# pscoro/JPEG-XL-Lossy-Image-Compression-Thesis

Measured on AMD Instinct MI355X. Metric: MPix/s VarDCT encode @ d1.0, 8K RGB, higher is better.
Workload: dtype f32; 1 GPU; 8k 7680x4320 RGB8 (synth_rgb8), VarDCT d1 e7, cjxl defaults (JXG_FLAGS_CJXL_DEFAULTS: Gaborish + EPF + masking AQ), proposals=0, ans-coded, 1 frame(s) per step, 2 distinct frames cycled, streaming entry points (jxg_submit_rgb8_device / jxg_receive, one host thread); global_batch=1, parallelism=frame-dp1

## Files before the change

jpeg-xl-lossy-image-compression-thesis_amd/csrc/jxg_ac.hip:

```cpp
#include "jxg_device.h"
#include "jxg_kernels.h"

namespace jxg {

constexpr int kAcCtxPad = (kAcCtx + 15) & ~15;
__constant__ __attribute__((aligned(16))) uint8_t c_cluster[kAcCtxPad];

constexpr int kAcThreads = 1024;

struct GroupGeom {
  int bx0, by0, gw, gh;
};
__device__ __forceinline__ uint32_t slot_group(const uint32_t* glist, uint32_t g0, uint32_t i) {
  return glist ? glist[i] : g0 + i;
}
__device__ __forceinline__ GroupGeom group_geom(const AcArgs& a, int g) {
  GroupGeom r;
  const int gx = g % (int)a.gxs, gy = g / (int)a.gxs;
  r.bx0 = gx * 32;
  r.by0 = gy * 32;
  r.gw = min(32, (int)a.bxs - r.bx0);
  r.gh = min(32, (int)a.bys - r.by0);
  return r;
}
// ... 429 lines not shown
}

__device__ __forceinline__ uint32_t wave_incl_scan(uint32_t v) {
  const int lane = threadIdx.x & 63;
#pragma unroll
  for (int d = 1; d < 64; d <<= 1) {
    const uint32_t t = __shfl_up(v, d);
    if (lane >= d) v += t;
  }
  return v;
}
__global__ __launch_bounds__(kAcThreads) void ac_emit_kernel(AcArgs a) {
  __shared__ uint32_t sCode[kMaxClusters * kAcTok];
  __shared__ __attribute__((aligned(16))) uint32_t sBits[kEmitLdsWords];
  __shared__ uint32_t sWave[kAcThreads / 64];
  const int g = (int)slot_group(a.glist, a.g0, blockIdx.x);
  for (int i = threadIdx.x; i < kMaxClusters * kAcTok; i += blockDim.x)
    sCode[i] = a.codes[(i / kAcTok) * kAlpha + (i % kAcTok)];
  for (int i = threadIdx.x; i < kEmitLdsWords / 4; i += blockDim.x)
    reinterpret_cast<uint4*>(sBits)[i] = make_uint4(0, 0, 0, 0);
  const uint32_t n = a.ntok[g * 3] + a.ntok[g * 3 + 1] + a.ntok[g * 3 + 2];
  const uint32_t* rec = a.tokens + (uint64_t)blockIdx.x * kGroupTokStride;
  uint32_t bt[kBands];
#pragma unroll
  for (int i = 0; i < kBands; i++) bt[i] = a.bandtok[g * kBands + i];
  constexpr int kWaves = kAcThreads / 64;
  const int lane = threadIdx.x & 63, wv = threadIdx.x >> 6;
  const uint32_t chunk = ((n + kWaves * 64 - 1) / (kWaves * 64)) * 64;
  const uint32_t lo = min(n, wv * chunk), hi = min(n, lo + chunk);
  __syncthreads();
  auto code_of = [&](uint32_t r) { return sCode[(r & 0xFF) * kAcTok + ((r >> 8) & 63)]; };
  uint32_t tot = 0;
  for (uint32_t k = lo + lane; k < hi; k += 64) {
    const uint32_t r = rec[rec_index(bt, k)];
    tot += (code_of(r) >> 16) + ((r >> 14) & 15);
  }
#pragma unroll
  for (int d = 32; d > 0; d >>= 1) tot += __shfl_xor(tot, d, 64);
  if (lane == 0) sWave[wv] = tot;
  __syncthreads();
  uint32_t run = 0, total = 0;
#pragma unroll
  for (int i = 0; i < kWaves; i++) {
    const uint32_t x = sWave[i];
    run += i < wv ? x : 0u;
    total += x;
  }
  const uint64_t base = a.base[g];
  const bool lds = total <= (uint32_t)kEmitLdsWords * 32u;
  if (!lds) {
    for (uint32_t i = threadIdx.x; i < (total + 31) / 32; i += blockDim.x) a.scratch[(base >> 5) + i] = 0;
    __threadfence();
    __syncthreads();
  }
  uint32_t* buf = lds ? sBits : a.scratch;
  const uint64_t bias = lds ? 0 : base;
  for (uint32_t k0 = lo; k0 < hi; k0 += 64) {
    const uint32_t k = k0 + lane;
    uint32_t len = 0, val = 0;
    if (k < hi) {
      const uint32_t r = rec[rec_index(bt, k)], cl = code_of(r);
      len = (cl >> 16) + ((r >> 14) & 15);
      val = (cl & 0xFFFFu) | ((r >> 18) << (cl >> 16));
    }
    const uint32_t incl = wave_incl_scan(len);
    if (len) {
      const uint64_t pos = bias + run + incl - len;
      const uint64_t w = pos >> 5;
      const uint32_t sh = (uint32_t)(pos & 31);
      atomicOr(&buf[w], val << sh);
      if (sh + len > 32) atomicOr(&buf[w + 1], val >> (32 - sh));
    }
    run += __shfl(incl, 63, 64);
  }
  if (lds) {
    __syncthreads();
    const uint32_t nw = (total + 31) / 32;
    uint32_t* dst = a.scratch + (base >> 5);
    for (uint32_t i = threadIdx.x; i < nw; i += blockDim.x) dst[i] = sBits[i];
  }
  if (threadIdx.x == 0) a.bits[g] = total;
}

#ifndef JXG_ANS_WAVES
#define JXG_ANS_WAVES 8
#endif
constexpr int kAnsWaves = JXG_ANS_WAVES;
__device__ __forceinline__ uint32_t wave_ror1(uint32_t x) {
  return (uint32_t)__builtin_amdgcn_mov_dpp((int)x, 0x13C, 0xF, 0xF, false);
}
__device__ __forceinline__ void ans_chain(const AnsArgs& a, uint32_t blk) {
  __shared__ uint32_t sSym[kAnsHists * 128];
  __shared__ uint32_t sInv[kAnsHists * 4096 / 2];
  __shared__ uint8_t sMap[136];
  const uint32_t* src = reinterpret_cast<const uint32_t*>(a.tab);
  for (uint32_t i = threadIdx.x; i < a.nhist * 128; i += blockDim.x) sSym[i] = src[i];
  for (uint32_t i = threadIdx.x; i < a.nhist * 2048; i += blockDim.x)
    sInv[i] = src[kAnsInvOff / 4 + i];
  for (uint32_t i = threadIdx.x; i < 136; i += blockDim.x) sMap[i] = a.tab[kAnsMapOff + i];
  __syncthreads();
  const uint8_t* inv = reinterpret_cast<const uint8_t*>(sInv);
  const uint32_t lane = threadIdx.x & 63;
  const uint32_t gi = __builtin_amdgcn_readfirstlane(blk * kAnsWaves + (threadIdx.x >> 6));
  if (gi >= a.n) return;
  const uint32_t slot = __builtin_amdgcn_readfirstlane(a.order[gi]);
  const uint32_t g = __builtin_amdgcn_readfirstlane(slot_group(a.glist, a.g0, slot));
  __builtin_amdgcn_s_setprio(3);
  const int n = (int)(a.ntok[g * 3] + a.ntok[g * 3 + 1] + a.ntok[g * 3 + 2]);
  const uint64_t b = (uint64_t)slot * kGroupTokStride;
  uint32_t bt[kBands];
#pragma unroll
  for (int i = 0; i < kBands; i++) bt[i] = a.bandtok[g * kBands + i];
  uint32_t k = 0x130u, v = 0;
  uint32_t rec = (int)lane < min(64, n) ? a.tokens[b + rec_index(bt, n - 1 - lane)] : 0u;
  for (int hi = n; hi > 0; hi -= 64) {
    const int cnt = min(64, hi);
    uint32_t f = 4096, base2 = 0;
    if ((int)lane < cnt) {
      const uint32_t h = sMap[rec & 0xFF], e = sSym[h * 128 + ((rec >> 8) & 63)];
      f = (e & 0xFFF) + 1;
      base2 = 2 * (h * 4096 + (e >> 12));
    }
    const uint32_t Fq = f << 8;
    const uint32_t nf2 = (uint32_t)(-(int)(2 * f));
    const double rcp = 1.0 / (double)f, hr = 0.5 * rcp;
    const int hn = hi - 64;
    const uint32_t nrec = (int)lane < min(64, hn) ? a.tokens[b + rec_index(bt, hn - 1 - lane)] : 0u;
    uint32_t X = 0;
    uint32_t xin = 0;
    auto step = [&](int s) {
      const uint32_t kin = wave_ror1(k);
      const uint32_t sh = kin >= Fq ? 16u : 0u;
      if (s > 0)
        asm("v_cndmask_b32_e64 %0, %1, %2, %3" : "=v"(X) : "v"(X), "v"(xin), "s"(1ull << (s - 1)));
      __builtin_amdgcn_sched_barrier(0);
      const uint32_t vin = wave_ror1(v);
      const uint32_t x = (kin << 12) + vin;
      const uint32_t xs = x >> sh;
      const uint32_t kk = (uint32_t)__builtin_fma((double)xs, rcp, hr);
      const uint32_t x2 = (xs << 1) + base2;
      uint32_t addr;
      asm("v_mad_i32_i24 %0, %1, %2, %3" : "=v"(addr) : "v"(kk), "v"(nf2), "v"(x2));
      v = *reinterpret_cast<const uint16_t*>(inv + addr);
      k = kk;
      xin = x;
      __builtin_amdgcn_sched_barrier(0);
    };
    if (cnt == 64) {
#pragma unroll
      for (int s = 0; s < 64; s++) step(s);
      asm("v_cndmask_b32_e64 %0, %1, %2, %3" : "=v"(X) : "v"(X), "v"(xin), "s"(1ull << 63));
    } else {
      for (int s = 0; s < cnt; s++) {
        const uint32_t kin = wave_ror1(k);
        const bool emit = kin >= Fq;
        const uint32_t t = (kin << 12) >> (emit ? 16 : 0);
        const double P = __builtin_fma((double)t, rcp, hr);
        const uint32_t C = 2 * t + base2;
        const uint32_t vin = wave_ror1(v);
        X = (int)lane == s ? (kin << 12) + vin : X;
        const uint32_t vv = emit ? 0u : vin;
        const uint32_t kk = (uint32_t)__builtin_fma((double)vv, rcp, P);
        const uint32_t addr = (uint32_t)((int)(2 * vv + C) - (int)(2 * f) * (int)kk);
        v = *reinterpret_cast<const uint16_t*>(inv + addr);
        k = kk;
      }
    }
    if ((int)lane < cnt) {
      const bool em = (X >> 20) >= f;
      const uint32_t raw = rec >> 18, nb = (rec >> 14) & 15;
      a.val[b + hi - 1 - lane] = em ? (X & 0xFFFFu) | raw << 16 : raw;
      a.len[b + hi - 1 - lane] = (uint8_t)(em ? nb + 16 : nb);
    }
    rec = nrec;
    if (hi <= 64) {
      const uint32_t kf = __builtin_amdgcn_readlane(k, cnt - 1);
      const uint32_t vf = __builtin_amdgcn_readlane(v, cnt - 1);
      if (lane == 0) a.state[g] = (kf << 12) + vf;
    }
  }
  if (n == 0 && lane == 0) a.state[g] = 0x130000u;
}
__global__ __launch_bounds__(kAnsWaves * 64) void ans_encode_kernel(Batch<AnsArgs> bt_) {
  ans_chain(bt_.a[blockIdx.z], blockIdx.x);
}
constexpr int kSumThreads = 1024;
__global__ __launch_bounds__(kSumThreads) void ans_sums_kernel(Batch<AnsArgs> bt_) {
  __shared__ uint32_t sC[kAnsMaxChunks];
  __shared__ uint32_t sTot[kSumThreads / 64];
  const AnsArgs& a = bt_.a[blockIdx.z];
  const uint32_t slot = blockIdx.x;
  if (slot >= a.n) return;
  const uint32_t g = slot_group(a.glist, a.g0, slot);
  const uint32_t n = a.ntok[g * 3] + a.ntok[g * 3 + 1] + a.ntok[g * 3 + 2];
  const uint32_t K = (n + 63) / 64;
  const uint64_t b = (uint64_t)slot * kGroupTokStride;
  const int lane = threadIdx.x & 63, wv = threadIdx.x >> 6;
  for (uint32_t q = threadIdx.x; q < K; q += kSumThreads) sC[q] = 0;
  __syncthreads();
  const uint32_t off = (64u - (n & 63u)) & 63u, r = n & 15u;
  const uint4* L = reinterpret_cast<const uint4*>(a.len + b);
  for (uint32_t w = threadIdx.x; w < (n + 15) / 16; w += kSumThreads) {
    const uint4 v = L[w];
    const uint32_t d[4] = {v.x, v.y, v.z, v.w};
    const uint32_t valid = min(16u, n - 16u * w);
    uint32_t lo = 0, hi = 0;
#pragma unroll
    for (uint32_t j = 0; j < 16; j++) {
      const uint32_t x = j < valid ? (d[j >> 2] >> (8 * (j & 3))) & 0xFFu : 0u;
      if (j < r) lo += x;
      else hi += x;
    }
    if (lo) atomicAdd(&sC[(16u * w + off) >> 6], lo);
    if (hi) atomicAdd(&sC[(16u * w + r + off) >> 6], hi);
  }
  __syncthreads();
  uint32_t* csum = a.csum + (uint64_t)slot * kAnsMaxChunks;
  uint32_t tot = 0;
  for (uint32_t q = threadIdx.x; q < K; q += kSumThreads) {
    const uint32_t c = sC[q];
    csum[q] = c;
    tot += c;
  }
#pragma unroll
  for (int m = 32; m > 0; m >>= 1) tot += __shfl_xor(tot, m, 64);
  if (lane == 0) sTot[wv] = tot;
  __syncthreads();
  uint32_t total = 32;
#pragma unroll
  for (int i = 0; i < kSumThreads / 64; i++) total += sTot[i];
  if (threadIdx.x == 0) a.bits[g] = total;
  uint32_t* dst = a.scratch + (a.base[g] >> 5);
  for (uint32_t i = threadIdx.x; i < (total + 31) / 32; i += kSumThreads) dst[i] = 0;
}
constexpr int kSegChunks = 64, kEmitThreads = 256;
constexpr int kSegWords = (kSegChunks * 64 * 29 + 31) / 32 + 2;
__global__ __launch_bounds__(kEmitThreads) void ans_emit_kernel(Batch<AnsArgs> bt_) {
  __shared__ __attribute__((aligned(16))) uint32_t sBits[kSegWords];
  __shared__ uint32_t sCs[kSegChunks + 1];
  __shared__ uint32_t sPre[kEmitThreads / 64];
  const AnsArgs& a = bt_.a[blockIdx.z];
  const uint32_t slot = blockIdx.x, seg = blockIdx.y;
  if (slot >= a.n) return;
  const uint32_t g = slot_group(a.glist, a.g0, slot);
  const uint32_t n = a.ntok[g * 3] + a.ntok[g * 3 + 1] + a.ntok[g * 3 + 2];
  const uint32_t K = (n + 63) / 64, q0 = seg * kSegChunks;
  const uint64_t base = a.base[g];
  if (seg == 0 && threadIdx.x == 0) a.scratch[base >> 5] = a.state[g];
  if (q0 >= K) return;
  const uint32_t q1 = min(K, q0 + kSegChunks);
  const uint32_t* csum = a.csum + (uint64_t)slot * kAnsMaxChunks;
  const int lane = threadIdx.x & 63, wv = threadIdx.x >> 6;
  uint32_t pre = 0;
  for (uint32_t q = threadIdx.x; q < q0; q += kEmitThreads) pre += csum[q];
#pragma unroll
  for (int d = 32; d > 0; d >>= 1) pre += __shfl_xor(pre, d, 64);
  if (lane == 0) sPre[wv] = pre;
  if (threadIdx.x <= kSegChunks) sCs[threadIdx.x] = q0 + threadIdx.x < q1 ? csum[q0 + threadIdx.x] : 0u;
  for (int i = threadIdx.x; i < kSegWords; i += kEmitThreads) sBits[i] = 0;
  __syncthreads();
  const uint64_t start = base + 32 + sPre[0] + sPre[1] + sPre[2] + sPre[3];
  const uint32_t sh0 = (uint32_t)(start & 31);
  uint32_t segbits = 0;
  for (uint32_t q = 0; q < q1 - q0; q++) segbits += sCs[q];
  auto chunk_lo = [&](uint32_t q) { return q == 0 ? 0u : n - 64u * (K - q); };
  const uint64_t b = (uint64_t)slot * kGroupTokStride;
  constexpr int kPerWave = kSegChunks / (kEmitThreads / 64);
  uint32_t run = sh0;
  for (int i = 0; i < wv * kPerWave; i++) run += sCs[i];
  for (int i = 0; i < kPerWave; i++) {
    const uint32_t q = q0 + (uint32_t)(wv * kPerWave + i);
    if (q >= q1) break;
    const uint32_t lo = chunk_lo(q), hi = chunk_lo(q + 1);
    const uint32_t k = lo + (uint32_t)lane;
    const uint32_t len = k < hi ? a.len[b + k] : 0u;
    const uint32_t val = k < hi ? a.val[b + k] : 0u;
    const uint32_t incl = wave_incl_scan(len);
    if (len) {
      const uint32_t pos = run + incl - len;
      const uint32_t w = pos >> 5, sh = pos & 31;
      atomicOr(&sBits[w], val << sh);
      if (sh + len > 32) atomicOr(&sBits[w + 1], val >> (32 - sh));
    }
    run += sCs[wv * kPerWave + i];
  }
  __syncthreads();
  const uint32_t nw = (sh0 + segbits + 31) / 32;
  uint32_t* dst = a.scratch + (start >> 5);
  for (uint32_t i = threadIdx.x; i < nw; i += kEmitThreads) {
    const uint32_t v = sBits[i];
    if (i == 0 || i == nw - 1) {
      if (v) atomicOr(&dst[i], v);
    } else {
      dst[i] = v;
    }
  }
}

void launch_ans(const AnsArgs* a, uint32_t k, hipStream_t s) {
  if (!k || !a[0].n) return;
  const Batch<AnsArgs> b = make_batch(a, k);
  uint32_t n = 0, maxtok = 0;
  for (uint32_t i = 0; i < k; i++) {
    n = max(n, a[i].n);
    maxtok = max(maxtok, a[i].max_tokens);
  }
  hipLaunchKernelGGL(ans_encode_kernel, dim3((n + kAnsWaves - 1) / kAnsWaves, 1, k),
                     dim3(kAnsWaves * 64), 0, s, b);
  hipLaunchKernelGGL(ans_sums_kernel, dim3(n, 1, k), dim3(kSumThreads), 0, s, b);
  const uint32_t nseg = (maxtok + kSegChunks * 64 - 1) / (kSegChunks * 64);
  if (nseg) hipLaunchKernelGGL(ans_emit_kernel, dim3(n, nseg, k), dim3(kEmitThreads), 0, s, b);
}

void launch_ac_hist(const AcArgs* a, uint32_t k, uint32_t ngroups, hipStream_t s, bool whole_group) {
  if (!ngroups || !k) return;
  if (whole_group)
    hipLaunchKernelGGL(ac_hist_kernel<32>, dim3(ngroups, 1, k), dim3(1024), 0, s, make_batch(a, k));
  else
    hipLaunchKernelGGL(ac_hist_kernel<8>, dim3(ngroups * kBands, 1, k), dim3(256), 0, s, make_batch(a, k));
}
void launch_ac_emit(const AcArgs& a, uint32_t ngroups, hipStream_t s) {
  if (ngroups) hipLaunchKernelGGL(ac_emit_kernel, dim3(ngroups), dim3(kAcThreads), 0, s, a);
}
hipError_t set_cluster_table(const uint8_t* tab, hipStream_t s) {
  return hipMemcpyToSymbolAsync(HIP_SYMBOL(c_cluster), tab, kAcCtx, 0, hipMemcpyHostToDevice, s);
}

}
```

jpeg-xl-lossy-image-compression-thesis_amd/csrc/jxg_host.cpp:

```cpp
#include <hip/hip_runtime.h>

#include <algorithm>
#include <atomic>
#include <chrono>
#include <cmath>
#include <condition_variable>
#include <cstdio>
#include <cstdlib>
#include <cstring>
#include <deque>
#include <functional>
#include <future>
#include <memory>
#include <mutex>
#include <new>
#include <thread>
#include <vector>

#include "../../include/jxg.h"
#include "jxg_bitstream.h"
#include "jxg_device.h"
#include "jxg_kernels.h"
#include "jxg_helpers.h"
#include "jxg_payload.h"
// ... 1153 lines not shown
    launch_ac_emit(J.aa, J.plan.ng(), s);
    JXG_HIP(hipGetLastError());
    JXG_HIP(hipMemcpyAsync(c->h_gbits.p, c->gbits.p, f.ngroups * 4, hipMemcpyDeviceToHost, s));
    JXG_HIP(hipEventRecord(c->ev[7], s));
  }

  JXG_HIP(hipEventSynchronize(c->ev[2]));
  const Clock::time_point t_lf = Clock::now();
  const size_t nlfcodes = (size_t)nstreams * 4 * kAlpha;
  JXG_HIP(c->h_lfcodes.ensure(nlfcodes));
  uint32_t* lfpacked = c->h_lfcodes.p;
  std::fill(lfpacked, lfpacked + nlfcodes, 0u);
  J.preA.assign(f.nlf, BitWriter());
  J.preB.assign(f.nlf, BitWriter());
  for (uint32_t lg = 0; lg < f.nlf; lg++) {
    if (!J.plan.owns_lf(lg)) continue;
    const uint32_t bx0 = (lg % f.lfxs) * 256, by0 = (lg / f.lfxs) * 256;
    const uint32_t bw = std::min(256u, f.bxs - bx0), bh = std::min(256u, f.bys - by0);
    for (int sidx = 0; sidx < 2; sidx++) {
      const uint32_t sid = lg * 2 + sidx;
      const int nleaves = sidx == 0 ? 3 : 4;
      std::vector<PrefixCode> lc(nleaves);
      for (int l = 0; l < nleaves; l++) {
        lc[l] = build_prefix_code(c->h_lfhist.p + ((size_t)sid * 4 + l) * kAlpha, kAlpha);
        for (int k = 0; k < kAlpha; k++) lfpacked[((size_t)sid * 4 + l) * kAlpha + k] = lc[l].packed(k);
      }
      if (sidx == 0) {
        J.preA[lg].put(2, 0);
        write_modular_prelude(J.preA[lg], kDcTree, 5, 3, lc);
      } else {
        J.preB[lg].put(ceil_log2(bw * bh), c->h_vcount.p[lg] - 1);
        write_modular_prelude(J.preB[lg], (J.lf >> 1) ? kMetaTreeEpf : kMetaTree, 7, 4, lc);
      }
    }
  }
  J.sbase.assign(nstreams, 0);
  cursor = 0;
  for (uint32_t i = 0; i < nstreams; i++) {
    J.sbase[i] = cursor;
    if (J.plan.owns_lf(i / 2)) cursor += ((uint64_t)c->h_sbound.p[i] + 63) & ~31ull;
  }
  const uint64_t lf_words = cursor / 32 + 2;
  JXG_HIP(c->h_sbase.ensure(J.sbase.size()));
  std::copy(J.sbase.begin(), J.sbase.end(), c->h_sbase.p);
  if (J.ans) {
    JXG_HIP(c->scratch.ensure(ac_words + lf_words));
    c->lf_scratch = c->scratch.p + ac_words;
    J.aa.scratch = c->scratch.p;
    JXG_HIP(hipMemcpyAsync(c->up.p + c->up_gbase, c->h_up.p + c->up_gbase,
                           c->up_bytes - c->up_gbase, hipMemcpyHostToDevice, s));
  } else {
    JXG_HIP(c->scratch_lf.ensure(lf_words));
    c->lf_scratch = c->scratch_lf.p;
    JXG_HIP(hipMemcpyAsync(c->up.p + c->up_lf, c->h_up.p + c->up_lf, c->up_bytes - c->up_lf,
                           hipMemcpyHostToDevice, s));
  }
  J.ms_codes = ms_ac_codes + ms_since(t_lf);
  return JXG_OK;
}

static void build_emit(Ctx* c, Job& J) {
  J.la.scratch = c->lf_scratch;
  if (!J.ans) return;
  AnsArgs& na = J.na;
  na = AnsArgs{};
  na.tokens = c->tokens.p;
  na.val = c->tval.p;
  na.len = c->tlen.p;
  na.ntok = c->ntok.p;
  na.bandtok = c->bandtok.p;
  na.tab = c->ans_tab.p;
  na.nhist = J.nhist_ans;
  na.state = c->ans_state.p;
  na.base = c->gbase.p;
  na.scratch = c->scratch.p;
  na.bits = c->gbits.p;
  na.g0 = J.plan.g0();
  na.n = J.plan.ng();
  na.glist = J.aa.glist;
  na.order = c->ans_order.p;
  na.csum = c->csum.p;
  na.max_tokens = J.max_tokens;
}
static jxg_status launch_emit(Ctx* const* cs, Job* const* js, uint32_t k) {
  if (!batch_ok(cs, js, k)) return JXG_ERR_INTERNAL;
  hipStream_t s = cs[0]->stream;
  const Job& J = *js[0];
  for (uint32_t i = 0; i < k; i++) build_emit(cs[i], *js[i]);
  if (J.ans) {
    const auto na = gather<AnsArgs>(js, k, [](Job& j) { return j.na; });
    launch_ans(na.data(), k, s);
    JXG_HIP(hipGetLastError());
  }
  const auto la = gather<LfArgs>(js, k, [](Job& j) { return j.la; });
  launch_lf_code(la.data(), k, J.nchunks, s);
  JXG_HIP(hipGetLastError());
  for (uint32_t i = 0; i < k; i++) {
    Ctx* c = cs[i];
    const Frame& f = js[i]->f;
    if (J.ans) {
      JXG_HIP(hipMemcpyAsync(c->h_bits.p, c->bits.p, ((size_t)f.ngroups + js[i]->nstreams) * 4,
                             hipMemcpyDeviceToHost, s));
      JXG_HIP(hipEventRecord(c->ev[7], s));
    } else {
      JXG_HIP(hipMemcpyAsync(c->h_sbits.p, c->stream_bits.p, js[i]->nstreams * 4,
                             hipMemcpyDeviceToHost, s));
    }
    JXG_HIP(hipEventRecord(c->ev[3], s));
  }
  return JXG_OK;
}
static jxg_status stage_emit(Ctx* c, Job& J, bool sync = true) {
  Job* jp = &J;
  jxg_status st = launch_emit(&c, &jp, 1);
  if (!st && sync) st = wait_emission(c, J);
  return st;
}

struct Piece {
  int arena;
  uint64_t src, nbits;
};
static jxg_status stage_concat(Ctx* c, Job& J, bool full, std::vector<uint32_t>* section_ids,
                               std::vector<uint32_t>* section_bytes, uint8_t** host_out,
                               size_t* out_bytes) {
  hipStream_t s = c->stream;
  const Frame& f = J.f;
  std::vector<std::vector<Piece>> sections;
  std::vector<uint32_t> ids;
  std::vector<uint32_t> chunk_words;
  auto add_chunk = [&](const BitWriter& bw) -> Piece {
    Piece p{1, (uint64_t)chunk_words.size() * 32, bw.bits()};
    auto wv = bw.words32();
    chunk_words.insert(chunk_words.end(), wv.begin(), wv.end());
    return p;
  };
  if (J.plan.rank == 0) {
    sections.push_back({add_chunk(J.lfglobal)});
    ids.push_back(0);
  }
  for (uint32_t lg = 0; lg < f.nlf; lg++) {
    if (!J.plan.owns_lf(lg)) continue;
    sections.push_back({add_chunk(J.preA[lg]), Piece{2, J.sbase[lg * 2], c->h_sbits.p[lg * 2]},
                        add_chunk(J.preB[lg]),
                        Piece{2, J.sbase[lg * 2 + 1], c->h_sbits.p[lg * 2 + 1]}});
    ids.push_back(1 + lg);
  }
  if (J.plan.rank == 0 && !J.presets) {
    sections.push_back({add_chunk(J.hfglobal)});
    ids.push_back(1 + f.nlf);
  }
  BitWriter sel;
  if (J.presets) sel.put(ceil_log2(J.plan.world), J.plan.rank);
  for (uint32_t g : J.plan.groups) {
    if (J.presets)
      sections.push_back({add_chunk(sel), Piece{0, J.gbase[g], c->h_gbits.p[g]}});
    else
      sections.push_back({Piece{0, J.gbase[g], c->h_gbits.p[g]}});
    ids.push_back(2 + f.nlf + g);
  }
  const bool single = full && f.ngroups == 1;
  std::vector<uint32_t> sizes;
  if (single) {
    uint64_t total = 0;
    for (auto& sec : sections)
      for (auto& p : sec) total += p.nbits;
    sizes.push_back((uint32_t)((total + 7) / 8));
  } else {
    for (auto& sec : sections) {
      uint64_t t = 0;
      for (auto& p : sec) t += p.nbits;
      sizes.push_back((uint32_t)((t + 7) / 8));
    }
  }
  std::vector<ConcatPiece> cps;
  uint64_t dst = 0, max_words = 0;
  auto emit_piece = [&](const Piece& p) {
    if (p.nbits) {
      cps.push_back({p.src, dst, p.nbits, (uint32_t)p.arena, 0});
      max_words = std::max<uint64_t>(max_words, (p.nbits + 31) / 32);
    }
    dst += p.nbits;
  };
  if (full) {
    BitWriter head;
    write_headers(head, J.w, J.h, J.lf);
    write_toc(head, sizes);
    emit_piece(add_chunk(head));
  }
  for (auto& sec : sections) {
    for (auto& p : sec) emit_piece(p);
    if (!single) dst = (dst + 7) & ~7ull;
  }
  dst = (dst + 7) & ~7ull;
  const size_t nbytes = (size_t)(dst / 8);
  const size_t out_words = (nbytes + 3) / 4 + 1;
  chunk_words.push_back(0);
// ... 295 lines not shown
      jxg_destroy(reinterpret_cast<jxg_ctx*>(c));
      return JXG_ERR_HIP;
    }
  *out = c;
  return JXG_OK;
}

static jxg_status encode_device(Ctx* c, const uint8_t* d_rgb, uint32_t w, uint32_t h,
                                size_t stride, jxg_buffer* out, Clock::time_point t_call) {
  if (pipe_busy(c)) return JXG_ERR_INVALID_ARG;
  Job J;
  jxg_status st = enc_launch(c, J, d_rgb, w, h, stride);
  if (st) return st;
  const bool split = J.f.ngroups > 1 && g_live_ctx.load() <= 1;
  if ((st = enc_codes(c, J, !split))) return st;
  return enc_finish(c, J, split, out, t_call);
}

#ifndef JXG_PIPE_CHAIN_GROUPS
#define JXG_PIPE_CHAIN_GROUPS 3570
#endif
constexpr uint32_t kPipeMaxLanes = 12, kPipeMinLanes = 4, kPipeChainGroups = JXG_PIPE_CHAIN_GROUPS;
static uint32_t hw_queues() {
  const char* e = std::getenv("GPU_MAX_HW_QUEUES");
  const long q = e && *e ? std::strtol(e, nullptr, 10) : 4;
  return (uint32_t)std::min<long>(32, std::max<long>(1, q));
}
#ifndef JXG_PIPE_BATCH_TILES
#define JXG_PIPE_BATCH_TILES 1280
#endif
constexpr uint32_t kPipeBatchTiles = JXG_PIPE_BATCH_TILES;
struct PipeShape {
  uint32_t lanes, batch;
  uint32_t frames() const { return lanes * batch; }
  uint32_t pending() const { return (lanes - 1) * batch + 1; }
};
static PipeShape pipe_shape(uint32_t ngroups, uint32_t ntiles, uint32_t cap) {
  const uint32_t want = (kPipeChainGroups + ngroups - 1) / std::max(1u, ngroups);
  uint32_t lmax = std::max(2u, std::min(kPipeMaxLanes, hw_queues() - 1));
  if (cap) lmax = std::min(lmax, cap);
  const uint32_t kt = ntiles <= kPipeBatchTiles ? kMaxBatch : 1u;
  const uint32_t k = std::min(kt, std::max(1u, (want + lmax - 1) / lmax));
  const uint32_t lanes = std::min(lmax, std::max(std::min(kPipeMinLanes, lmax), (want + k - 1) / k));
  return PipeShape{lanes, k};
}
struct PipeDone {
  jxg_buffer buf;
  jxg_stats stats;
  hipEvent_t ev;
};
struct PipeBatch;
struct PipeFrame {
  Ctx* lane = nullptr;
  Ctx* owner = nullptr;
  std::shared_ptr<PipeBatch> batch;
  Job J;
  int phase = 0;
  bool shard = false;
  Clock::time_point t0;
  const uint8_t* src = nullptr;
  uint32_t w = 0, h = 0, rank = 0, world = 1;
  size_t stride = 0;
  std::future<jxg_status> codes;
};
struct PipeBatch {
  Ctx* owner = nullptr;
  uint32_t w = 0, h = 0, rank = 0, world = 1;
  bool shard = false;
  std::vector<PipeFrame*> frames;
  std::atomic<int> left{0};
  std::atomic<int> err{JXG_OK};
};
static jxg_status pipe_codes(PipeFrame* fr) {
  PipeBatch& B = *fr->batch;
  jxg_status st = stage_codes(fr->lane, fr->J);
  if (st) B.err.store(st);
  if (B.left.fetch_sub(1) == 1 && !B.err.load()) {
    std::vector<Ctx*> cs;
    std::vector<Job*> js;
    for (PipeFrame* q : B.frames) {
      cs.push_back(q->lane);
      js.push_back(&q->J);
    }
    const jxg_status e = launch_emit(cs.data(), js.data(), (uint32_t)cs.size());
    if (e) B.err.store(e);
  }
  return st;
}
static jxg_status pipe_join_codes(PipeFrame& fr) {
  jxg_status st = JXG_OK;
  if (fr.codes.valid()) {
    st = fr.codes.get();
    fr.phase = 2;
  }
  if (!st && fr.batch) st = (jxg_status)fr.batch->err.load();
  return st;
}
constexpr int kPipeHelpers = 6;

struct Pipe {
  std::vector<std::unique_ptr<PipeFrame>> inflight;
  std::vector<PipeDone> done;
  std::vector<hipEvent_t> evfree;
  std::vector<std::unique_ptr<PipeFrame>> ready;
  uint64_t submitted = 0;
  int mode = 0;
  uint32_t depth = 0;
  std::shared_ptr<PipeBatch> open;
  std::deque<hipEvent_t> writes;
  std::unique_ptr<Helpers> helpers;
  ~Pipe() {
    for (auto& d : done)
      if (d.ev) {
        (void)hipEventSynchronize(d.ev);
        (void)hipEventDestroy(d.ev);
      }
    for (hipEvent_t e : evfree) (void)hipEventDestroy(e);
  }
};
static jxg_status pipe_done_wait(Pipe& p, PipeDone& d) {
  if (!d.ev) return JXG_OK;
  const hipError_t e = hipEventSynchronize(d.ev);
  p.evfree.push_back(d.ev);
  d.ev = nullptr;
  return e == hipSuccess ? JXG_OK : JXG_ERR_HIP;
}
static void pipe_drop_done(Pipe& p) {
  for (auto& d : p.done) {
    (void)pipe_done_wait(p, d);
    jxg_buffer_free(&d.buf);
  }
  p.done.clear();
}
static bool pipe_busy(const Ctx* c) {
  return c->pipe && (!c->pipe->inflight.empty() || !c->pipe->done.empty() ||
                     !c->pipe->ready.empty());
}

static jxg_status ensure_lanes(Ctx* c, uint32_t extra) {
  while (c->lanes.size() < extra) {
    Ctx* l = nullptr;
    const jxg_status st = ctx_new_lane(c->params, &l);
    if (st) return st;
    c->lanes.emplace_back(l);
  }
  return JXG_OK;
}
static jxg_status ensure_slots(Ctx* L, uint32_t k) {
  while (L->slots.size() + 1 < k) {
    Ctx* q = new (std::nothrow) Ctx();
    if (!q) return JXG_ERR_OOM;
    q->params = L->params;
    q->owned_lane = true;
    q->shared_stream = true;
    q->stream = L->stream;
    L->slots.emplace_back(q);
    for (auto& e : q->ev)
      if (make_event(&e, 0) != hipSuccess) return JXG_ERR_HIP;
  }
  return JXG_OK;
}
static Ctx* lane_slot(Ctx* L, uint32_t i) { return i == 0 ? L : L->slots[i - 1].get(); }

static void pipe_abort(Ctx* c) {
  Pipe& p = *c->pipe;
  p.open.reset();
  for (auto& fr : p.inflight) (void)pipe_join_codes(*fr);
// ... 1259 lines not shown
```

jpeg-xl-lossy-image-compression-thesis_amd/csrc/jxg_kernels.h:

```cpp
#pragma once
#include <cmath>
#include <hip/hip_runtime.h>
#include <stddef.h>
#include <stdint.h>

namespace jxg {

constexpr uint32_t kMaxBatch = 4;
template <class A>
struct Batch {
  A a[kMaxBatch];
};
template <class A>
inline Batch<A> make_batch(const A* a, uint32_t k) {
  Batch<A> b{};
  for (uint32_t i = 0; i < k && i < kMaxBatch; i++) b.a[i] = a[i];
  return b;
}

struct FrontArgs {
  const uint8_t* rgb;
  uint32_t w, h;
  size_t stride;
  uint32_t bxs, bys, xp, yp, tiles_x;
// ... 67 lines not shown
constexpr size_t kBigPlanes = 3 * 65536;
constexpr size_t kBigTabW = 0, kBigTabSd = 3 * 122880, kBigTabIw = 6 * 122880,
                 kBigTabLeeC = 7 * 122880, kBigTabLeeS = kBigTabLeeC + 9 * 128,
                 kBigTabLlfP = kBigTabLeeS + 9 * 256, kBigTabLlfIb = kBigTabLlfP + 6 * 32,
                 kBigTabFloats = kBigTabLlfIb + 6 * 32 * 32;
struct BigArgs {
  MergeArgs m;
  const float* tab;
  const uint16_t* nat;
  float* scratch;
  uint32_t slots;
  float* cost;
  uint32_t* work;
  uint32_t* kinds;
  const uint32_t* glist;
  uint32_t g0, ng, gxs;
};
hipError_t launch_big(const BigArgs* a, uint32_t k, hipStream_t s);

struct VbArgs {
  const uint8_t* acs;
  uint32_t bxs, bys, lfxs;
  const uint8_t* lf_mine;
  uint32_t* vb;
  uint32_t* count;
};

struct HomogArgs {
  const float* xyb;
  uint32_t xsize, ysize;
  size_t stride, plane;
  float distance;
  int h1_int;
  float* r3;
  uint8_t* type;
};

struct AcArgs {
  const uint8_t* acs;
  const int16_t* ac;
  const uint16_t* nz;
  uint32_t bxs, bys, gxs;
  uint32_t g0;
  const uint32_t* glist;
  uint32_t* hist;
  uint32_t* bound;
  uint32_t* ntok;
  const uint32_t* codes;
  const uint64_t* base;
  uint32_t* scratch;
  uint32_t* bits;
  uint32_t* tokens;
  uint32_t* bandtok;
};
constexpr uint64_t kGroupTokStride = 1024ull * 3 * 64;
constexpr uint64_t kBandTokStride = 256ull * 3 * 64;

#ifndef JXG_ANS_HISTS
#define JXG_ANS_HISTS 8
#endif
constexpr uint32_t kAnsHists = JXG_ANS_HISTS;
constexpr uint32_t kAnsInvOff = kAnsHists * 128 * 4;
constexpr uint32_t kAnsMapOff = kAnsInvOff + kAnsHists * 4096 * 2;
constexpr uint32_t kAnsTabBytes = kAnsMapOff + 136;
struct AnsArgs {
  const uint32_t* tokens;
  uint32_t* val;
  uint8_t* len;
  const uint32_t* ntok;
  const uint32_t* bandtok;
  const uint8_t* tab;
  uint32_t nhist;
  uint32_t* state;
  const uint64_t* base;
  uint32_t* scratch;
  uint32_t* bits;
  uint32_t g0, n;
  const uint32_t* glist;
  const uint32_t* order;
  uint32_t* csum;
  uint32_t max_tokens;
};
constexpr uint32_t kAnsMaxChunks = (uint32_t)(kGroupTokStride / 64);
void launch_ans(const AnsArgs* a, uint32_t k, hipStream_t s);

constexpr uint32_t kLfSeg = 256;
struct LfRow {
  uint32_t lg;
  uint16_t stream;
  uint16_t chan;
  uint32_t y, x0, width;
  uint32_t sid;
};
constexpr uint32_t kLfChunkSamples = 4096, kLfChunkRows = 64, kLfPer = 16;
struct LfChunk {
  uint32_t row0, nrows, sid, nsamp;
};
struct LfArgs {
  const LfRow* rows;
  const LfChunk* chunks;
  const int32_t* dc;
  const uint8_t* acs;
  const uint8_t* qf;
  const uint32_t* vb;
  const uint32_t* vcount;
  uint32_t bxs, bys, lfxs;
  const int8_t* cmap;
  uint32_t tiles_x, ntiles_all;
  uint32_t* hist;
  uint32_t* sbound;
  const uint32_t* codes;
  uint64_t* status;
  const uint32_t* stream_chunks;
  const uint64_t* stream_base;
  uint32_t* stream_bits;
  uint32_t* scratch;
};

struct ConcatPiece {
  uint64_t src_bit;
  uint64_t dst_bit;
  uint64_t nbits;
  uint32_t arena;
  uint32_t pad;
};

inline float dist_weight(int c, int area, float w) {
  static const float kW0[3] = {3150.0f, 560.0f, 512.0f};
  return (float)(std::sqrt((double)area / 64.0) * ((double)kW0[c] / (double)w));
}
hipError_t set_front_constants(const float lut[256], const float wts[5][3][64], hipStream_t s);
void launch_front(const FrontArgs* a, uint32_t k, uint32_t tiles_x, uint32_t tiles_y, hipStream_t s);
void launch_front_list(const FrontArgs* a, uint32_t k, uint32_t ntiles, hipStream_t s);
struct PackArgs {
  uint8_t* acs;
  uint8_t* qf;
  int32_t* dc;
  uint32_t bxs, bys, gxs;
  int8_t* cmap;
  uint32_t tiles_x, tiles_y;
  uint8_t* xbuf;
  const uint32_t* list;
  uint32_t n;
};
void launch_pack(const PackArgs& a, hipStream_t s);
struct ScatterPiece {
  uint64_t src, dst;
  uint32_t len, wg0;
};
constexpr int kMaxScatterPieces = 64;
struct ScatterArgs {
  const uint8_t* src;
  uint8_t* dst;
  uint32_t n;
  ScatterPiece p[kMaxScatterPieces];
};
void launch_scatter(const ScatterArgs& a, uint32_t nwg, hipStream_t s);
void launch_unpack(const PackArgs& a, hipStream_t s);
void launch_homog(const HomogArgs& a, uint32_t tiles_x, uint32_t tiles_y, hipStream_t s);
void launch_ac_hist(const AcArgs* a, uint32_t k, uint32_t ngroups, hipStream_t s,
                    bool whole_group = false);
void launch_ac_emit(const AcArgs& a, uint32_t ngroups, hipStream_t s);
void launch_lf_hist(const LfArgs* a, uint32_t k, uint32_t nchunks, hipStream_t s);
void launch_lf_code(const LfArgs* a, uint32_t k, uint32_t nchunks, hipStream_t s);
hipError_t set_cluster_table(const uint8_t* tab, hipStream_t s);
hipError_t set_merge_constants(const float* llf_p , const float* llf_ib ,
                         hipStream_t s);
// ... 62 lines not shown
```

Baseline: 9534 MPix/s.

## Encode 64 ANS chains per workgroup with helper waves staging tokens through LDS

Adds a new ANS encode kernel for the streamed pipeline. Each workgroup handles 64 groups, one group per lane of a single chain wave. Six helper waves prefetch token records, pre-decode them into compact words in double-buffered LDS tiles, and write out the val/len outputs. The per-symbol division is done with a precomputed double reciprocal and FMA, and table constants are packed into LDS. The old one-chain-per-wave kernel is kept as the non-streamed path. The aim is to hide global-memory latency and the serial work around the dependent state chain, at the cost of large LDS use, barrier sync per block, and imbalance when chain lengths in a workgroup differ.

```diff
diff --git a/jpeg-xl-lossy-image-compression-thesis_amd/csrc/jxg_ac.hip b/jpeg-xl-lossy-image-compression-thesis_amd/csrc/jxg_ac.hip
--- a/jpeg-xl-lossy-image-compression-thesis_amd/csrc/jxg_ac.hip
+++ b/jpeg-xl-lossy-image-compression-thesis_amd/csrc/jxg_ac.hip
@@ -535,14 +535,193 @@
   if (threadIdx.x == 0) a.bits[g] = total;
 }
 
-#ifndef JXG_ANS_WAVES
-#define JXG_ANS_WAVES 8
-#endif
-constexpr int kAnsWaves = JXG_ANS_WAVES;
+constexpr int kAnsWgWaves = 8;
+constexpr int kAnsHelpers = 6;
+constexpr int kAnsPieces = (64 + kAnsHelpers - 1) / kAnsHelpers;
+constexpr int kAnsBlk = 64;
+constexpr int kAnsRow = 65;
+constexpr uint32_t kAnsIdle = kAnsHists * 64;
+struct AnsConst {
+  double rcp;
+  uint32_t nf2;
+  uint32_t base2;
+};
+struct AnsChainP {
+  int n;
+  uint32_t slot;
+  uint32_t c1, c2, c3;
+  uint32_t g;
+  uint32_t pad[2];
+};
+struct AnsLds {
+  AnsConst c[kAnsIdle + 1];
+  uint16_t ent[256];
+  uint32_t inv[kAnsHists * 4096 / 2];
+  uint32_t ea[2][kAnsBlk * kAnsRow];
+  uint32_t x[2][kAnsBlk * kAnsRow];
+  AnsChainP ch[64];
+  int T;
+};
+__device__ __forceinline__ void ans_chain(const AnsArgs& a, uint32_t blk) {
+  __shared__ __attribute__((aligned(16))) AnsLds L;
+  const uint32_t c0 = blk * 64;
+  if (c0 >= a.n) return;
+  const uint32_t* src = reinterpret_cast<const uint32_t*>(a.tab);
+  for (uint32_t i = threadIdx.x; i < a.nhist * 512; i += blockDim.x)
+    reinterpret_cast<uint4*>(L.inv)[i] = reinterpret_cast<const uint4*>(src + kAnsInvOff / 4)[i];
+  for (uint32_t i = threadIdx.x; i <= kAnsIdle; i += blockDim.x) {
+    uint32_t f = 4096, row = 0;
+    if (i < a.nhist * 64) {
+      const uint32_t e = src[(i >> 6) * 128 + (i & 63)];
+      f = (e & 0xFFF) + 1;
+      row = (i >> 6) * 4096 + (e >> 12);
+    }
+    L.c[i].rcp = 1.0 / (double)f;
+    L.c[i].nf2 = (uint32_t)(-(int)(2 * f));
+    L.c[i].base2 = 2 * row;
+  }
+  for (uint32_t i = threadIdx.x; i < 256; i += blockDim.x)
+    L.ent[i] = (uint16_t)(i < 136 ? min((uint32_t)a.tab[kAnsMapOff + i], kAnsHists - 1) * 64 * 16
+                                  : kAnsIdle * 16);
+  const uint32_t lane = threadIdx.x & 63, wave = threadIdx.x >> 6;
+  if (wave == 0) {
+    AnsChainP P = {0, 0, 0, 0, 0, ~0u, {0, 0}};
+    if (c0 + lane < a.n) {
+      P.slot = a.order[c0 + lane];
+      P.g = slot_group(a.glist, a.g0, P.slot);
+      P.n = (int)(a.ntok[P.g * 3] + a.ntok[P.g * 3 + 1] + a.ntok[P.g * 3 + 2]);
+      P.c1 = a.bandtok[P.g * kBands];
+      P.c2 = P.c1 + a.bandtok[P.g * kBands + 1];
+      P.c3 = P.c2 + a.bandtok[P.g * kBands + 2];
+    }
+    L.ch[lane] = P;
+    int m = P.n;
+#pragma unroll
+    for (int d = 32; d > 0; d >>= 1) m = max(m, __shfl_xor(m, d, 64));
+    if (lane == 0) L.T = m + 1;
+  }
+  __syncthreads();
+  const int NB = (L.T + kAnsBlk - 1) / kAnsBlk;
+  const uint8_t* inv = reinterpret_cast<const uint8_t*>(L.inv);
+  const uint8_t* cst = reinterpret_cast<const uint8_t*>(L.c);
+  const int h = (wave & 3) ? (int)(wave >> 2) * 3 + (int)(wave & 3) - 1 : -1;
+  const uint32_t hs = lane;
+  auto word_of = [&](uint32_t rec) {
+    return ((uint32_t)L.ent[rec & 0xFF] + ((rec >> 4) & 0x3F0)) | ((rec >> 14) & 15) | (rec >> 18) << 14;
+  };
+  auto record = [&](const AnsChainP& P, int i) {
+    const uint32_t u = (uint32_t)i;
+    const uint32_t j = (u >= P.c1 ? 1u : 0u) + (u >= P.c2 ? 1u : 0u) + (u >= P.c3 ? 1u : 0u);
+    const uint32_t lo = u >= P.c3 ? P.c3 : u >= P.c2 ? P.c2 : u >= P.c1 ? P.c1 : 0u;
+    return a.tokens[(uint64_t)P.slot * kGroupTokStride + j * (uint32_t)kBandTokStride + (u - lo)];
+  };
+  constexpr uint32_t kIdleRec = 0xFFu;
+  auto fetch = [&](int b, uint32_t* R) {
+#pragma unroll
+    for (int j = 0; j < kAnsPieces; j++) {
+      const int q = h + kAnsHelpers * j;
+      R[j] = kIdleRec;
+      if (q < 64) {
+        const AnsChainP P = L.ch[q];
+        const int i = P.n - 1 - (b * kAnsBlk + (int)hs);
+        if (i >= 0) R[j] = record(P, i);
+      }
+    }
+  };
+  auto fill = [&](int b, const uint32_t* R) {
+#pragma unroll
+    for (int j = 0; j < kAnsPieces; j++) {
+      const int q = h + kAnsHelpers * j;
+      if (q < 64) L.ea[b & 1][hs * kAnsRow + q] = word_of(R[j]);
+    }
+  };
+  auto unstage = [&](int b, uint32_t* X, uint32_t* RC) {
+#pragma unroll
+    for (int j = 0; j < kAnsPieces; j++) {
+      const int q = h + kAnsHelpers * j;
+      X[j] = RC[j] = 0;
+      if (q < 64) {
+        X[j] = L.x[b & 1][hs * kAnsRow + q];
+        RC[j] = L.ea[b & 1][hs * kAnsRow + q];
+      }
+    }
+  };
+  auto flush = [&](int b, const uint32_t* X, const uint32_t* RC) {
+#pragma unroll
+    for (int j = 0; j < kAnsPieces; j++) {
+      const int q = h + kAnsHelpers * j;
+      if (q < 64) {
+        const AnsChainP P = L.ch[q];
+        const int i = P.n - 1 - (b * kAnsBlk + (int)hs);
+        const uint32_t x = X[j], w = RC[j];
+        if (i >= 0) {
+          const uint32_t nf2 = reinterpret_cast<const AnsConst*>(cst + (w & 0x3FF0))->nf2;
+          const bool em = (x >> 12) >= (uint32_t)__mul24((int)nf2, -128);
+          const uint32_t raw = w >> 14, nb = w & 15;
+          const uint64_t o = (uint64_t)P.slot * kGroupTokStride + (uint32_t)i;
+          a.val[o] = em ? (x & 0xFFFFu) | raw << 16 : raw;
+          a.len[o] = (uint8_t)(em ? nb + 16 : nb);
+        } else if (i == -1 && P.g != ~0u) {
+          a.state[P.g] = x;
+        }
+      }
+    }
+  };
+  uint32_t k = 0x130u, v = 0;
+  auto chain_block = [&](int b) {
+    const uint32_t* eas = L.ea[b & 1] + lane;
+    uint32_t* xo = L.x[b & 1] + lane;
+    AnsConst Cn = *reinterpret_cast<const AnsConst*>(cst + (eas[0] & 0x3FF0));
+#pragma unroll
+    for (int s = 0; s < kAnsBlk; s++) {
+      const AnsConst C = Cn;
+      if (s + 1 < kAnsBlk) Cn = *reinterpret_cast<const AnsConst*>(cst + (eas[(s + 1) * kAnsRow] & 0x3FF0));
+      const double hr = 0.5 * C.rcp;
+      const uint32_t Fq = (uint32_t)__mul24((int)C.nf2, -128);
+      const uint32_t sh = k >= Fq ? 16u : 0u;
+      const uint32_t x = (k << 12) + v;
+      const uint32_t xs = x >> sh;
+      const uint32_t kk = (uint32_t)__builtin_fma((double)xs, C.rcp, hr);
+      const uint32_t x2 = (xs << 1) + C.base2;
+      uint32_t addr;
+      asm("v_mad_i32_i24 %0, %1, %2, %3" : "=v"(addr) : "v"(kk), "v"(C.nf2), "v"(x2));
+      v = *reinterpret_cast<const uint16_t*>(inv + addr);
+      k = kk;
+      xo[s * kAnsRow] = x;
+    }
+  };
+  if (wave == 0) __builtin_amdgcn_s_setprio(3);
+  uint32_t R[kAnsPieces], X[kAnsPieces], RC[kAnsPieces];
+  if (h >= 0) {
+    fetch(0, R);
+    fill(0, R);
+    fetch(1, R);
+  }
+  __syncthreads();
+  for (int b = 0; b < NB; b++) {
+    if (wave == 0) {
+      chain_block(b);
+    } else if (h >= 0) {
+      if (b > 0) unstage(b - 1, X, RC);
+      fill(b + 1, R);
+      fetch(b + 2, R);
+      if (b > 0) flush(b - 1, X, RC);
+    }
+    __syncthreads();
+  }
+  if (h >= 0) {
+    unstage(NB - 1, X, RC);
+    flush(NB - 1, X, RC);
+  }
+}
+__global__ __launch_bounds__(kAnsWgWaves * 64) void ans_encode_kernel(Batch<AnsArgs> bt_) {
+  ans_chain(bt_.a[blockIdx.z], blockIdx.x);
+}
+constexpr int kAnsDiagWaves = 8;
 __device__ __forceinline__ uint32_t wave_ror1(uint32_t x) {
   return (uint32_t)__builtin_amdgcn_mov_dpp((int)x, 0x13C, 0xF, 0xF, false);
 }
-__device__ __forceinline__ void ans_chain(const AnsArgs& a, uint32_t blk) {
+__device__ __forceinline__ void ans_chain_diag(const AnsArgs& a, uint32_t blk) {
   __shared__ uint32_t sSym[kAnsHists * 128];
   __shared__ uint32_t sInv[kAnsHists * 4096 / 2];
   __shared__ uint8_t sMap[136];
@@ -554,7 +733,7 @@
   __syncthreads();
   const uint8_t* inv = reinterpret_cast<const uint8_t*>(sInv);
   const uint32_t lane = threadIdx.x & 63;
-  const uint32_t gi = __builtin_amdgcn_readfirstlane(blk * kAnsWaves + (threadIdx.x >> 6));
+  const uint32_t gi = __builtin_amdgcn_readfirstlane(blk * kAnsDiagWaves + (threadIdx.x >> 6));
   if (gi >= a.n) return;
   const uint32_t slot = __builtin_amdgcn_readfirstlane(a.order[gi]);
   const uint32_t g = __builtin_amdgcn_readfirstlane(slot_group(a.glist, a.g0, slot));
@@ -634,8 +813,8 @@
   }
   if (n == 0 && lane == 0) a.state[g] = 0x130000u;
 }
-__global__ __launch_bounds__(kAnsWaves * 64) void ans_encode_kernel(Batch<AnsArgs> bt_) {
-  ans_chain(bt_.a[blockIdx.z], blockIdx.x);
+__global__ __launch_bounds__(kAnsDiagWaves * 64) void ans_encode_diag_kernel(Batch<AnsArgs> bt_) {
+  ans_chain_diag(bt_.a[blockIdx.z], blockIdx.x);
 }
 constexpr int kSumThreads = 1024;
 __global__ __launch_bounds__(kSumThreads) void ans_sums_kernel(Batch<AnsArgs> bt_) {
@@ -750,7 +929,7 @@
   }
 }
 
-void launch_ans(const AnsArgs* a, uint32_t k, hipStream_t s) {
+void launch_ans(const AnsArgs* a, uint32_t k, hipStream_t s, bool streamed) {
   if (!k || !a[0].n) return;
   const Batch<AnsArgs> b = make_batch(a, k);
   uint32_t n = 0, maxtok = 0;
@@ -758,8 +937,11 @@
     n = max(n, a[i].n);
     maxtok = max(maxtok, a[i].max_tokens);
   }
-  hipLaunchKernelGGL(ans_encode_kernel, dim3((n + kAnsWaves - 1) / kAnsWaves, 1, k),
-                     dim3(kAnsWaves * 64), 0, s, b);
+  if (streamed)
+    hipLaunchKernelGGL(ans_encode_kernel, dim3((n + 63) / 64, 1, k), dim3(kAnsWgWaves * 64), 0, s, b);
+  else
+    hipLaunchKernelGGL(ans_encode_diag_kernel, dim3((n + kAnsDiagWaves - 1) / kAnsDiagWaves, 1, k),
+                       dim3(kAnsDiagWaves * 64), 0, s, b);
   hipLaunchKernelGGL(ans_sums_kernel, dim3(n, 1, k), dim3(kSumThreads), 0, s, b);
   const uint32_t nseg = (maxtok + kSegChunks * 64 - 1) / (kSegChunks * 64);
   if (nseg) hipLaunchKernelGGL(ans_emit_kernel, dim3(n, nseg, k), dim3(kEmitThreads), 0, s, b);
diff --git a/jpeg-xl-lossy-image-compression-thesis_amd/csrc/jxg_host.cpp b/jpeg-xl-lossy-image-compression-thesis_amd/csrc/jxg_host.cpp
--- a/jpeg-xl-lossy-image-compression-thesis_amd/csrc/jxg_host.cpp
+++ b/jpeg-xl-lossy-image-compression-thesis_amd/csrc/jxg_host.cpp
@@ -1259,14 +1259,14 @@
   na.csum = c->csum.p;
   na.max_tokens = J.max_tokens;
 }
-static jxg_status launch_emit(Ctx* const* cs, Job* const* js, uint32_t k) {
+static jxg_status launch_emit(Ctx* const* cs, Job* const* js, uint32_t k, bool streamed) {
   if (!batch_ok(cs, js, k)) return JXG_ERR_INTERNAL;
   hipStream_t s = cs[0]->stream;
   const Job& J = *js[0];
   for (uint32_t i = 0; i < k; i++) build_emit(cs[i], *js[i]);
   if (J.ans) {
     const auto na = gather<AnsArgs>(js, k, [](Job& j) { return j.na; });
-    launch_ans(na.data(), k, s);
+    launch_ans(na.data(), k, s, streamed);
     JXG_HIP(hipGetLastError());
   }
   const auto la = gather<LfArgs>(js, k, [](Job& j) { return j.la; });
@@ -1289,7 +1289,7 @@
 }
 static jxg_status stage_emit(Ctx* c, Job& J, bool sync = true) {
   Job* jp = &J;
-  jxg_status st = launch_emit(&c, &jp, 1);
+  jxg_status st = launch_emit(&c, &jp, 1, false);
   if (!st && sync) st = wait_emission(c, J);
   return st;
 }
@@ -1751,7 +1751,7 @@
       cs.push_back(q->lane);
       js.push_back(&q->J);
     }
-    const jxg_status e = launch_emit(cs.data(), js.data(), (uint32_t)cs.size());
+    const jxg_status e = launch_emit(cs.data(), js.data(), (uint32_t)cs.size(), true);
     if (e) B.err.store(e);
   }
   return st;
diff --git a/jpeg-xl-lossy-image-compression-thesis_amd/csrc/jxg_kernels.h b/jpeg-xl-lossy-image-compression-thesis_amd/csrc/jxg_kernels.h
--- a/jpeg-xl-lossy-image-compression-thesis_amd/csrc/jxg_kernels.h
+++ b/jpeg-xl-lossy-image-compression-thesis_amd/csrc/jxg_kernels.h
@@ -173,7 +173,7 @@
   uint32_t max_tokens;
 };
 constexpr uint32_t kAnsMaxChunks = (uint32_t)(kGroupTokStride / 64);
-void launch_ans(const AnsArgs* a, uint32_t k, hipStream_t s);
+void launch_ans(const AnsArgs* a, uint32_t k, hipStream_t s, bool streamed);
 
 constexpr uint32_t kLfSeg = 256;
 struct LfRow {
```

Result: faster. 10200 MPix/s (median of 6 runs) (+7.0%).
